# sangminwoo/Temporal-Span-Proposal-Network-VidVRD

Hardware: AMD Instinct MI355X
Metric: tracklet-pairs/sec scored (N=32, T=150, D=2048) (higher is better)
Workload: dtype f32

## Files before the change

### include/tspn_mi355x.h

```cpp
#ifndef TSPN_MI355X_H
#define TSPN_MI355X_H

#include <stddef.h>
#include <stdint.h>

#ifdef __cplusplus
extern "C" {
#endif

#define TSPN_ABI_VERSION 7

enum {
  TSPN_OK = 0,
  TSPN_EINVAL = -1,
  TSPN_EUNSUPPORTED = -2,
  TSPN_EWORKSPACE = -3,
  TSPN_ELAUNCH = -4,
  TSPN_EDEVICE = -5
};

#define TSPN_STATUS_WORDS 16
enum {
  TSPN_STATUS_FAULT = 0,
  TSPN_STATUS_FAULT_INFO = 1,
// ... 62 lines not shown
int tspn_traj_iou_tail_f64(const double* a, const int32_t* len_a, const double* b, int64_t U, int64_t N,
                           int64_t L, float* out, void* stream);

int tspn_pair_index_i64(int64_t N, int64_t base, int64_t* pairs, void* stream);

int tspn_pair_gather_f32(const float* feats, const float* boxes, int64_t NT, int64_t T,
                         int64_t D, const int64_t* pairs, int64_t P,
                         float* out_feat, float* out_geom, void* stream);

int tspn_pack_conv3_f32(const float* W, int64_t M, int64_t Cin, int64_t split,
                        float* packed, void* stream);

int tspn_conv3_f32(const float* x, int64_t B, int64_t Cin, int64_t T,
                   const float* packed, int64_t M, const float* bias, int relu,
                   float* y, void* stream);

int tspn_conv3_tc_f32(const float* x, int64_t B, int64_t T, int64_t Cin,
                      const float* packed, int64_t M, const float* bias, int relu,
                      float* y, void* stream);

int tspn_pack_conv3_wino63_frag_f32(const float* W, int64_t M, int64_t Cin, int64_t split, float* frag,
                                    void* stream);
size_t tspn_conv3_tc_wino63_workspace_bytes(int64_t B, int64_t T, int64_t Cin);
int tspn_conv3_tc_wino63_f32(const float* x, int64_t B, int64_t T, int64_t Cin, const float* frag,
                             int64_t M, const float* bias, int relu, float* y,
                             void* workspace, size_t workspace_bytes, void* stream);
int tspn_conv3_tc_wino63_set_piece_form(int form);

size_t tspn_pack_conv3_wino63_f16x3_elements(int64_t M, int64_t Cin, int64_t split);
int tspn_pack_conv3_wino63_f16x3(const float* W, int64_t M, int64_t Cin, int64_t split, int16_t* packed, void* stream);
size_t tspn_conv3_tc_wino63_f16x3_workspace_bytes(int64_t B, int64_t T, int64_t Cin, int64_t M);
int tspn_conv3_tc_wino63_f16x3(const float* x, int64_t B, int64_t T, int64_t Cin, const int16_t* packed,
                               int64_t M, const float* bias, int relu, float* y,
                               void* workspace, size_t workspace_bytes, void* stream);
int tspn_conv3_tc_wino63_f16x3_set_tail_split(int on);
int tspn_conv3_tc_wino63_f16x3_input_form(int64_t NT, int64_t T, int64_t Cin, int cus);
int tspn_conv3_tc_wino63_f16x3_set_input_form(int form);
int tspn_conv3_tc_wino63_f16x3_input(const float* x, int64_t B, int64_t T, int64_t Cin, int64_t M, void* split_input,
                                     size_t split_input_bytes, float* fbar, uint64_t* hot_slots, void* stream);


int tspn_heads_f32(int mode, const float* a, const float* b, int64_t lda,
                   const int64_t* ia, const int64_t* ib, int64_t idx_stride, const float* bias,
                   const float* Wh, const float* bh, int64_t H,
                   int64_t P, int64_t C, int64_t T, float* out, void* stream);

int tspn_heads_pairgrid_f32(const float* y, int64_t B, int64_t N, int64_t C, int64_t T,
                            const float* Wh, const float* bh, int64_t H, float* out,
                            void* stream);

size_t tspn_heads_pairgrid_f16x3_split_bytes(int64_t C, int64_t H);
int tspn_heads_pairgrid_f16x3_set_force_exact(int on);
int tspn_heads_pair_f16x3_set_diag_skip(int on);
int tspn_heads_pairgrid_f16x3(const float* y, int64_t ldt, int64_t B, int64_t N, int64_t C, int64_t T,
                              const float* Wh, const float* bh, int64_t H, void* split_buf, size_t split_bytes,
                              float* out, void* stream);

int tspn_temporal_mean_f32(const float* x, int64_t R, int64_t T, int64_t Cdim,
                           int layout_tc, float* out, void* stream);
int tspn_temporal_sum_f32(const float* x, int64_t R, int64_t T, int64_t Cdim, float* out, void* stream);

int tspn_pair_rows_f32(const float* src, int64_t NT, int64_t D, const int64_t* pairs,
                       int64_t P, float* out, void* stream);

int tspn_transpose_td_f32(const float* x, int64_t R, int64_t T, int64_t D, float* out,
                          void* stream);

size_t tspn_decode_topk_workspace_bytes(int64_t S, int64_t P, int64_t topk_pair);
int tspn_decode_topk_f32(const float* rel_logit, const int64_t* pairs,
                         const float* cls_sub, const float* cls_obj, int64_t ld,
                         int64_t seg_rows, int64_t row_mul, int64_t S, int64_t P, int64_t K,
                         int64_t NO, int64_t topk_pair, int64_t topk_seg,
                         float* out_score, int64_t* out_triplet, int64_t* out_pair_tid,
                         void* workspace, size_t workspace_bytes, void* stream);

int tspn_decode_spans_f32(const float* heads, int64_t P, int64_t A, int64_t T,
                          const float* sizes_host, int64_t top_k, double nms_threshold,
                          int64_t pre_nms, int64_t* out_anchor, int64_t* out_span,
                          float* out_span_f, float* out_score, int64_t* out_count, void* stream);

typedef struct tspn_fused_desc {
  int64_t B, N, T, D;
  int64_t A, K;
  const float* feats;
  const int64_t* pairs;
  int64_t P;
  int64_t canonical_pairs;
  const float* conv_packed;
  int64_t conv_algo;
  const float* conv_bias;
  const float* head_w;
  const float* head_b;
  const float* cls_w;
  const float* cls_b;
  float* out_heads;
  float* out_logits;
  void* workspace;
  size_t workspace_bytes;
  void* ev_conv_begin;
  void* ev_conv_end;
  void* ev_logits_ready;
  const float* conv_weight;
  int64_t conv_check;
} tspn_fused_desc;

size_t tspn_forward_fused_workspace_bytes(const tspn_fused_desc* d);
// ... 210 lines not shown
```

### temporal-span-proposal-network-vidvrd_amd/_abi.py

```python
import ctypes
import os
import re
import threading

HERE = os.path.dirname(os.path.abspath(__file__))
ROOT = os.path.dirname(HERE)
LIB_PATH = os.environ.get("TSPN_LIB_PATH") or os.path.join(HERE, "libtspn_mi355x.so")
HEADER_PATH = os.path.join(ROOT, "include", "tspn_mi355x.h")

ABI_VERSION = 7
TSPN_OK = 0
TSPN_EINVAL = -1
TSPN_EUNSUPPORTED = -2
TSPN_EWORKSPACE = -3
TSPN_ELAUNCH = -4
TSPN_EDEVICE = -5
STATUS_WORDS = 16
STATUS_FAULT, STATUS_FAULT_INFO, STATUS_CONV_ERR, STATUS_CONV_CHECKS = 0, 1, 2, 3
FAULT_HANDOVER = 1
CONV_CHECK_HOT_OFFSET, CONV_CHECK_SCRATCH_BYTES = 256, 256 + 256 * 64
GEOM_CHANNELS = 8
CONV_DIRECT, CONV_WINOGRAD63, CONV_WINOGRAD63_F16X3 = 0, 1, 2

_c_f32p = ctypes.c_void_p
# ... 18 lines not shown
        ("conv_weight", _vp), ("conv_check", _i64),
    ]


class FusedBf16Desc(ctypes.Structure):
    _fields_ = [
        ("B", _i64), ("N", _i64), ("T", _i64), ("D", _i64),
        ("A", _i64), ("K", _i64),
        ("feats", _vp), ("pairs", _vp), ("P", _i64),
        ("conv_packed", _vp), ("conv_bias", _vp),
        ("head_packed", _vp), ("head_b", _vp),
        ("cls_w", _vp), ("cls_b", _vp),
        ("out_heads", _vp), ("out_logits", _vp),
        ("workspace", _vp), ("workspace_bytes", _sz),
        ("ev_conv_begin", _vp), ("ev_conv_end", _vp), ("ev_logits_ready", _vp),
    ]


PROTOTYPES = {
    "tspn_version": (_int, []),
    "tspn_fused_desc_size": (_sz, []),
    "tspn_fused_bf16_desc_size": (_sz, []),
    "tspn_last_error": (ctypes.c_char_p, []),
    "tspn_error_string": (ctypes.c_char_p, [_int]),
    "tspn_status_attach": (_int, [_vp]),
    "tspn_status_fault": (_int, []),
    "tspn_status_clear": (_int, []),
    "tspn_status_selftest": (_int, [_vp, _vp]),
    "tspn_conv3_spot_check_f32": (_int, [_vp, _i64, _i64, _i64, _vp, _i64, _i64, _i64, _vp, _int, _vp, _i64, _vp, _i64, _vp]),
    "tspn_predicate_head_workspace_bytes": (_sz, [_i64, _i64, _i64]),
    "tspn_predicate_head_f32": (_int, [_vp, _i64, _i64, _i64, _vp, _vp, _i64, _vp, _int, _vp, _sz, _vp]),
    "tspn_predicate_head_norm_workspace_bytes": (_sz, [_i64, _i64, _i64, _i64, _i64, _i64]),
    "tspn_predicate_head_norm_f32": (_int, [_vp, _i64, _i64, _i64, _vp, _vp, _i64, _i64, _i64, _i64, _vp, _int,
                                            _vp, _sz, _vp]),
    "tspn_feature_preprocess_f32": (_int, [_vp, _i64, _i64, _i64, _i64, _i64, _i64, _vp]),
    "tspn_proposal_pair_filter_i64": (_int, [_vp, _vp, _vp, _vp, _i64, _vp, _vp, _vp, _vp]),
    "tspn_gather_rows_f32": (_int, [_vp, _i64, _i64, _vp, _i64, _i64, _vp, _vp]),
    "tspn_ppn_pair_matrix_topk_f32": (_int, [_vp, _i64, _i64, _i64, _i64, _i64,
                                             _vp, _vp, _vp, _vp, _vp, _vp, _vp, _vp,
                                             _i64, _vp, _vp, _vp]),
    "tspn_traj_iou_f32": (_int, [_vp, _i64, _vp, _i64, _i64, _i64, _vp, _vp]),
    "tspn_traj_iou_tail_f64": (_int, [_vp, _vp, _vp, _i64, _i64, _i64, _vp, _vp]),
    "tspn_pair_index_i64": (_int, [_i64, _i64, _vp, _vp]),
    "tspn_pair_gather_f32": (_int, [_vp, _vp, _i64, _i64, _i64, _vp, _i64, _vp, _vp, _vp]),
    "tspn_pack_conv3_f32": (_int, [_vp, _i64, _i64, _i64, _vp, _vp]),
    "tspn_conv3_f32": (_int, [_vp, _i64, _i64, _i64, _vp, _i64, _vp, _int, _vp, _vp]),
    "tspn_conv3_tc_f32": (_int, [_vp, _i64, _i64, _i64, _vp, _i64, _vp, _int, _vp, _vp]),
    "tspn_heads_f32": (_int, [_int, _vp, _vp, _i64, _vp, _vp, _i64, _vp, _vp, _vp, _i64, _i64, _i64,
                              _i64, _vp, _vp]),
    "tspn_heads_pairgrid_f32": (_int, [_vp, _i64, _i64, _i64, _i64, _vp, _vp, _i64, _vp, _vp]),
    "tspn_heads_pairgrid_f16x3_split_bytes": (_sz, [_i64, _i64]),
    "tspn_heads_pairgrid_f16x3_set_force_exact": (_int, [_int]),
    "tspn_heads_pair_f16x3_set_diag_skip": (_int, [_int]),
    "tspn_heads_pairgrid_f16x3": (_int, [_vp, _i64, _i64, _i64, _i64, _i64, _vp, _vp, _i64, _vp, _sz, _vp, _vp]),
    "tspn_temporal_mean_f32": (_int, [_vp, _i64, _i64, _i64, _int, _vp, _vp]),
    "tspn_temporal_sum_f32": (_int, [_vp, _i64, _i64, _i64, _vp, _vp]),
    "tspn_pair_rows_f32": (_int, [_vp, _i64, _i64, _vp, _i64, _vp, _vp]),
    "tspn_transpose_td_f32": (_int, [_vp, _i64, _i64, _i64, _vp, _vp]),
    "tspn_decode_topk_workspace_bytes": (_sz, [_i64, _i64, _i64]),
    "tspn_decode_topk_f32": (_int, [_vp, _vp, _vp, _vp, _i64, _i64, _i64, _i64, _i64, _i64, _i64, _i64, _i64,
                                    _vp, _vp, _vp, _vp, _sz, _vp]),
    "tspn_decode_spans_f32": (_int, [_vp, _i64, _i64, _i64, ctypes.POINTER(ctypes.c_float), _i64,
                                     ctypes.c_double, _i64, _vp, _vp, _vp, _vp, _vp, _vp]),
    "tspn_forward_fused_workspace_bytes": (_sz, [ctypes.POINTER(FusedDesc)]),
    "tspn_forward_fused_f32": (_int, [ctypes.POINTER(FusedDesc), _vp]),
    "tspn_temporal_encoder_heads_f32": (_int, [_vp, _i64, _i64, _i64, _vp, _vp, _vp, _vp, _i64,
                                               _vp, _vp, _vp]),
    "tspn_pack_conv2d_f32": (_int, [_vp, _i64, _i64, _i64, _i64, _vp, _vp]),
    "tspn_conv2d_nhwc_f32": (_int, [_vp, _i64, _i64, _i64, _i64, _vp, _i64, _i64, _i64, _i64, _i64, _vp, _vp,
                                    _int, _vp, _vp]),
    "tspn_pack_conv2d_frag_f32": (_int, [_vp, _i64, _i64, _i64, _i64, _vp, _vp]),
    "tspn_conv2d_nhwc_frag_f32": (_int, [_vp, _i64, _i64, _i64, _i64, _vp, _i64, _i64, _i64, _i64, _i64, _vp, _vp,
                                         _int, _vp, _vp]),
    "tspn_pack_conv2d_frag_bf16": (_int, [_vp, _i64, _i64, _i64, _i64, _vp, _vp]),
    "tspn_conv2d_nhwc_bf16": (_int, [_vp, _i64, _i64, _i64, _i64, _vp, _i64, _i64, _i64, _i64, _i64, _vp, _vp,
                                     _int, _vp, _vp]),
    "tspn_roi_align_nhwc_f32": (_int, [_vp, _i64, _i64, _i64, _i64, _vp, _i64, _i64, ctypes.c_float, _int, _int,
                                       _int, _vp, _vp]),
    "tspn_pack_conv2d_frag_cin4_f32": (_int, [_vp, _i64, _i64, _i64, _i64, _vp, _vp]),
    "tspn_conv2d_nhwc_cin4_f32": (_int, [_vp, _i64, _i64, _i64, _vp, _i64, _i64, _i64, _i64, _i64, _vp, _int, _vp, _vp]),
    "tspn_max_pool_nhwc_f32": (_int, [_vp, _i64, _i64, _i64, _i64, _i64, _i64, _i64, _vp, _int, _vp]),
    "tspn_bottleneck_tail_bf16": (_int, [_vp, _i64, _i64, _i64, _i64, _vp, _vp, _vp, _vp, _vp, _vp, _vp]),
    "tspn_bottleneck_block_bf16": (_int, [_vp, _i64, _i64, _i64, _i64, _vp, _vp, _vp, _vp, _vp, _vp, _vp, _vp]),
    "tspn_bottleneck_block_proj_bf16": (_int, [_vp, _i64, _i64, _i64, _i64, _i64, _i64, _vp, _vp, _vp, _vp, _vp, _vp, _vp, _vp,
                                               _vp, _vp]),
    "tspn_bottleneck_block_res_bf16": (_int, [_vp, _i64, _i64, _i64, _i64, _i64, _i64, _vp, _vp, _vp, _vp, _vp, _vp, _vp, _vp, _vp]),
    "tspn_bottleneck_tail_io_bf16": (_int, [_vp, _i64, _i64, _i64, _i64, _vp, _vp, _vp, _vp, _vp, _vp, _vp]),
    "tspn_bottleneck_tail_pipe_bf16": (_int, [_vp, _i64, _i64, _i64, _i64, _vp, _vp, _vp, _vp, _vp, _vp, _i64, _vp]),
    "tspn_bottleneck_tail_next_bf16": (_int, [_vp, _i64, _i64, _i64, _i64, _vp, _vp, _vp, _vp, _vp, _vp, _vp, _vp, _vp, _vp]),
    "tspn_stem_bf16_workspace_bytes": (_sz, [_i64, _i64, _i64]),
    "tspn_pack_stem_bf16": (_int, [_vp, _i64, _vp, _vp]),
    "tspn_stem_conv_bf16": (_int, [_vp, _i64, _i64, _i64, _vp, _i64, _vp, _vp, _sz, _vp, _vp]),
    "tspn_max_pool_nhwc_bf16": (_int, [_vp, _i64, _i64, _i64, _i64, _i64, _i64, _i64, _vp, _vp]),
    "tspn_stem_pool_bf16": (_int, [_vp, _i64, _i64, _i64, _vp, _i64, _vp, _vp, _sz, _vp, _vp]),
    "tspn_roi_align_nhwc_bf16": (_int, [_vp, _i64, _i64, _i64, _i64, _vp, _i64, _i64, ctypes.c_float, _int, _int,
                                        _int, _vp, _vp]),
    "tspn_roi_align_nhwc_f32_bf16out": (_int, [_vp, _i64, _i64, _i64, _i64, _vp, _i64, _i64, ctypes.c_float, _int, _int,
                                               _int, _vp, _vp]),
    "tspn_pack_conv3_wino63_frag_f32": (_int, [_vp, _i64, _i64, _i64, _vp, _vp]),
    "tspn_conv3_tc_wino63_workspace_bytes": (_sz, [_i64, _i64, _i64]),
    "tspn_conv3_tc_wino63_f32": (_int, [_vp, _i64, _i64, _i64, _vp, _i64, _vp, _int, _vp, _vp, _sz, _vp]),
    "tspn_conv3_tc_wino63_set_piece_form": (_int, [_int]),
    "tspn_pack_conv3_wino63_f16x3_elements": (_sz, [_i64, _i64, _i64]),
    "tspn_pack_conv3_wino63_f16x3": (_int, [_vp, _i64, _i64, _i64, _vp, _vp]),
    "tspn_conv3_tc_wino63_f16x3_workspace_bytes": (_sz, [_i64, _i64, _i64, _i64]),
    "tspn_conv3_tc_wino63_f16x3": (_int, [_vp, _i64, _i64, _i64, _vp, _i64, _vp, _int, _vp, _vp, _sz, _vp]),
# ... 103 lines not shown
```

### temporal-span-proposal-network-vidvrd_amd/csrc/pairf16/tspn_heads_pair_f16x3.hip

```cpp
#include "tspn_common.h"
#include "tspn_device.h"

#include <type_traits>

namespace {
using namespace tspn_dev;

constexpr int PF_S = 8, PF_O = 8, PF_T = 32, PF_CK = 32;
constexpr int PF_ROWS = PF_S + PF_O;
constexpr int PF_STAGE = PF_ROWS * PF_CK * PF_T;
constexpr int PF_THREADS = 64 * PF_S;
constexpr size_t PF_SMEM = sizeof(float) * 2 * PF_STAGE;
constexpr int PF_HDR_BYTES = 256;
constexpr int PF_KSTEP_BYTES = 2 * 64 * 16;
constexpr float PF_LO = 2048.f, PF_LO_INV = 1.f / 2048.f;
constexpr float PF_RANGE = 16384.f;

typedef _Float16 f16x2 __attribute__((ext_vector_type(2)));

std::atomic<int> g_force_exact{0};
std::atomic<int> g_diag_skip{1};

__device__ __forceinline__ unsigned split_lo(unsigned h2, float as0, float as1) {
  unsigned d;
  const float neg = -PF_LO;
  asm("v_fma_mixlo_f16 %0, %1, %2, %3 op_sel_hi:[1,0,0]" : "=v"(d) : "v"(h2), "s"(neg), "v"(as0));
  asm("v_fma_mixhi_f16 %0, %1, %2, %3 op_sel:[1,0,0] op_sel_hi:[1,0,0]" : "+v"(d) : "v"(h2), "s"(neg), "v"(as1));
  return d;
}

__global__ __launch_bounds__(1024) void pairf16_scale_kernel(const float* __restrict__ Wh, int C, int H,
                                                            unsigned* __restrict__ hdr) {
  __shared__ unsigned bad_s[16];
  const int lane = threadIdx.x & 63, h = threadIdx.x >> 6;
  float mx = 0.f;
  bool finite = true;
  auto take = [&](float w, float& m) {
    const float a = fabsf(w);
    finite = finite && (a < __builtin_inff());
    m = fmaxf(m, a);
  };
  if (h < H && (reinterpret_cast<uintptr_t>(Wh) & 15) == 0) {
    const float4* row = reinterpret_cast<const float4*>(Wh + (int64_t)h * C);
    const int n4 = C >> 2;
    float m[4] = {0.f, 0.f, 0.f, 0.f};
    int c = lane;
    for (; c + 192 < n4; c += 256) {
      float4 v[4];
#pragma unroll
      for (int u = 0; u < 4; ++u) v[u] = row[c + 64 * u];
#pragma unroll
      for (int u = 0; u < 4; ++u) { take(v[u].x, m[u]); take(v[u].y, m[u]); take(v[u].z, m[u]); take(v[u].w, m[u]); }
    }
    for (; c < n4; c += 64) {
      const float4 v = row[c];
      take(v.x, m[0]); take(v.y, m[0]); take(v.z, m[0]); take(v.w, m[0]);
    }
    mx = fmaxf(fmaxf(m[0], m[1]), fmaxf(m[2], m[3]));
  } else if (h < H) {
    for (int c = lane; c < C; c += 64) take(Wh[(int64_t)h * C + c], mx);
  }
#pragma unroll
  for (int o = 32; o > 0; o >>= 1) mx = fmaxf(mx, __shfl_xor(mx, o, 64));
  const bool all_finite = __all(finite);
  int e = 0;
  (void)frexpf(mx, &e);
  const bool bad = h < H && (!all_finite || !(mx >= 0x1p-100f) || e > 100);
  if (lane == 0) {
    bad_s[h] = bad ? 1u : 0u;
    hdr[1 + h] = __float_as_uint((h < H && !bad) ? ldexpf(1.f, e) : 1.f);
  }
  __syncthreads();
  if (threadIdx.x == 0) {
    unsigned f = 0;
    for (int i = 0; i < 16; ++i) f |= bad_s[i];
    hdr[0] = f;
  }
  if (threadIdx.x >= 17 && threadIdx.x < PF_HDR_BYTES / 4) hdr[threadIdx.x] = 0;
}

__global__ __launch_bounds__(64) void pairf16_pack_kernel(const float* __restrict__ Wh, int C, int H,
                                                         const unsigned* __restrict__ hdr, u32x4* __restrict__ frag) {
  const int lane = threadIdx.x, h = lane & 15, kg = lane >> 4;
  const float scale = 1.f / __uint_as_float(hdr[1 + h]);
  unsigned hi[4], lo[4];
#pragma unroll
  for (int ip = 0; ip < 4; ++ip) {
    f16x2 wh, wl;
#pragma unroll
    for (int e = 0; e < 2; ++e) {
      const int c = blockIdx.x * PF_CK + kg + 4 * (2 * ip + e);
      const float w = (h < H) ? Wh[(int64_t)h * C + c] * scale : 0.f;
      const _Float16 a = (_Float16)w;
      wh[e] = a;
      wl[e] = (_Float16)((w - (float)a) * PF_LO);
    }
    hi[ip] = __builtin_bit_cast(unsigned, wh);
    lo[ip] = __builtin_bit_cast(unsigned, wl);
  }
  frag[(int64_t)blockIdx.x * 128 + lane] = u32x4{hi[0], hi[1], hi[2], hi[3]};
  frag[(int64_t)blockIdx.x * 128 + 64 + lane] = u32x4{lo[0], lo[1], lo[2], lo[3]};
}

__device__ __noinline__ void exact_tile(const float* __restrict__ y, int64_t ldt, int C, int T, int N, int H,
                                        const float* __restrict__ Wh, const float* __restrict__ bh,
                                        float* __restrict__ out, int64_t b, int sb, int ob, int t0) {
  const int t = t0 + (threadIdx.x & 31);
  if (t >= T) return;
  for (int idx = threadIdx.x >> 5; idx < PF_S * PF_O * H; idx += PF_THREADS / 32) {
    const int pair = idx / H, h = idx - pair * H;
    const int s = sb * PF_S + (pair >> 3), o = ob * PF_O + (pair & 7);
    if (s >= N || o >= N || s == o) continue;
    const float* up = y + ((b * N + s) * 2 * (int64_t)C) * ldt + t;
    const float* vp = y + ((b * N + o) * 2 * (int64_t)C + C) * ldt + t;
    const float* w = Wh + (int64_t)h * C;
    float sum = 0.f;
    for (int c = 0; c < C; ++c) sum = __builtin_fmaf(w[c], tspn::relu_f32(up[c * ldt] + vp[c * ldt]), sum);
    const int64_t p = b * N * (int64_t)(N - 1) + (int64_t)s * (N - 1) + o - (o > s ? 1 : 0);
    out[(p * H + h) * (int64_t)T + t] = sum + (bh ? bh[h] : 0.f);
  }
}

__global__ __launch_bounds__(PF_THREADS, 1) void heads_pair_f16x3_kernel(
    const float* __restrict__ y, int64_t ldt, int C, int T, int N, int H, const float* __restrict__ Wh,
    const float* __restrict__ bh, const unsigned* __restrict__ hdr, const u32x4* __restrict__ frag,
    float* __restrict__ out, int ntb, int nob, int nsb, int64_t ngroups, int force_exact, int diag_skip) {
  extern __shared__ __attribute__((aligned(16))) char smem_raw[];
  float* S = reinterpret_cast<float*>(smem_raw);

  const int tid = threadIdx.x;
  const int lane = tid & 63;
  const int wave = __builtin_amdgcn_readfirstlane(tid >> 6);
  const int j = lane & 15, kg = lane >> 4;
  int sb, ob;
  const int64_t G = pair_stage_group(blockIdx.x, nsb, nob, sb, ob);
  if (G >= ngroups) return;
  const int64_t b = G / ntb;
  const int t0 = (int)(G - b * ntb) * PF_T;
  const int64_t rowlen = 2 * (int64_t)C * ldt;

  if (force_exact | (int)hdr[0]) {
    exact_tile(y, ldt, C, T, N, H, Wh, bh, out, b, sb, ob, t0);
    return;
  }

  const __amdgpu_buffer_rsrc_t rsrc_y = buffer_rsrc(y + b * N * rowlen, (int)(unsigned)((int64_t)N * rowlen * 4));
  unsigned voff[2];
  const unsigned loff = (unsigned)((lane >> 3) * ldt + min((int64_t)t0 + (lane & 7) * 4, ldt - 4));
#pragma unroll
  for (int r = 0; r < 2; ++r) {
    const int row = 2 * wave + r;
    const int local = row < PF_S ? sb * PF_S + row : ob * PF_O + (row - PF_S);
    const int64_t trk = min(local, N - 1);
    voff[r] = (unsigned)((trk * rowlen + (row < PF_S ? 0 : (int64_t)C * ldt) + loff) * 4);
  }
  const int piece_bytes = (int)(8 * ldt * 4);
  int y_soff = 0;
  auto stage = [&](int buf) {
#pragma unroll
    for (int r = 0; r < 2; ++r) {
#pragma unroll
      for (int q = 0; q < 4; ++q)
        bglds16(rsrc_y, voff[r], y_soff + q * piece_bytes, S + buf * PF_STAGE + ((2 * wave + r) * PF_CK + 8 * q) * PF_T);
    }
    y_soff += 4 * piece_bytes;
  };

  f32x4 acc_hi[PF_O][2], acc_lo[PF_O][2];
#pragma unroll
  for (int o = 0; o < PF_O; ++o) {
#pragma unroll
    for (int cb = 0; cb < 2; ++cb) acc_hi[o][cb] = acc_lo[o][cb] = f32x4{0.f, 0.f, 0.f, 0.f};
  }

  const int nk = C / PF_CK;
  stage(0);
  u32x4 wh = frag[lane], wl = frag[64 + lane];
  asm volatile("s_waitcnt vmcnt(0)" ::: "memory");
  __syncthreads();
  const float* urow = S + (wave * PF_CK + kg) * PF_T + 2 * j;
  const float* vrow = S + (PF_S * PF_CK + kg) * PF_T + 2 * j;
  const float* trow = vrow + wave * PF_CK * PF_T;
  float mu = 0.f, mv = 0.f;
  const bool diag = diag_skip && sb == ob;
  auto kloop = [&](auto diag_c) {
    constexpr bool DIAG = decltype(diag_c)::value;
    constexpr int NS = DIAG ? PF_O - 1 : PF_O;
    for (int k = 0; k < nk; ++k) {
      const int buf = k & 1;
      u32x4 whn = wh, wln = wl;
      if (k + 1 < nk) {
        stage(buf ^ 1);
        whn = frag[(int64_t)(k + 1) * 128 + lane];
        wln = frag[(int64_t)(k + 1) * 128 + 64 + lane];
      }
// ... 35 lines not shown
#pragma unroll
          for (int cb = 0; cb < 2; ++cb) {
            unsigned ph[4], pl[4];
#pragma unroll
            for (int ip = 0; ip < 4; ++ip) {
              const f16x2 h = __builtin_convertvector(f32x2{a[2 * ip][cb], a[2 * ip + 1][cb]}, f16x2);
              ph[ip] = __builtin_bit_cast(unsigned, h);
              pl[ip] = split_lo(ph[ip], as[2 * ip][cb], as[2 * ip + 1][cb]);
            }
            gh[cb] = u32x4{ph[0], ph[1], ph[2], ph[3]};
            gl[cb] = u32x4{pl[0], pl[1], pl[2], pl[3]};
          }
        }
        if (o > 0) {
          const f16x8 h0 = __builtin_bit_cast(f16x8, fh[0]), h1 = __builtin_bit_cast(f16x8, fh[1]);
          const f16x8 l0 = __builtin_bit_cast(f16x8, fl[0]), l1 = __builtin_bit_cast(f16x8, fl[1]);
          acc_hi[o - 1][0] = __builtin_amdgcn_mfma_f32_16x16x32_f16(a_hi, h0, acc_hi[o - 1][0], 0, 0, 0);
          acc_lo[o - 1][0] = __builtin_amdgcn_mfma_f32_16x16x32_f16(a_hi, l0, acc_lo[o - 1][0], 0, 0, 0);
          acc_hi[o - 1][1] = __builtin_amdgcn_mfma_f32_16x16x32_f16(a_hi, h1, acc_hi[o - 1][1], 0, 0, 0);
          acc_lo[o - 1][1] = __builtin_amdgcn_mfma_f32_16x16x32_f16(a_hi, l1, acc_lo[o - 1][1], 0, 0, 0);
          acc_lo[o - 1][0] = __builtin_amdgcn_mfma_f32_16x16x32_f16(a_lo, h0, acc_lo[o - 1][0], 0, 0, 0);
          acc_lo[o - 1][1] = __builtin_amdgcn_mfma_f32_16x16x32_f16(a_lo, h1, acc_lo[o - 1][1], 0, 0, 0);
        }
        if (o > 0 && o < NS) {
#define TSPN_G                                         \
  __builtin_amdgcn_sched_group_barrier(0x008, 1, 0);   \
  __builtin_amdgcn_sched_group_barrier(0x100, 2, 0);   \
  __builtin_amdgcn_sched_group_barrier(0x002, 10, 0);
          TSPN_G TSPN_G TSPN_G TSPN_G TSPN_G TSPN_G
#undef TSPN_G
        }
        __builtin_amdgcn_sched_barrier(0);
#pragma unroll
        for (int cb = 0; cb < 2; ++cb) {
          fh[cb] = gh[cb];
          fl[cb] = gl[cb];
        }
#pragma unroll
        for (int i = 0; i < 8; ++i) v[i] = vn[i];
      }
      wh = whn;
      wl = wln;
      asm volatile("s_waitcnt vmcnt(0)" ::: "memory");
      __syncthreads();
    }
  };
  if (diag) kloop(std::true_type{});
  else kloop(std::false_type{});

  const int tA = t0 + 2 * j;
  const int s = sb * PF_S + wave;
  const bool bad = tA < T && ((s < N && !(mu <= PF_RANGE)) || (ob * PF_O + wave < N && !(mv <= PF_RANGE)));
  if (__syncthreads_or(bad)) {
    exact_tile(y, ldt, C, T, N, H, Wh, bh, out, b, sb, ob, t0);
    return;
  }

  if (tA >= T || s >= N) return;
  float inv[4], bias[4];
#pragma unroll
  for (int r = 0; r < 4; ++r) {
    const int h = 4 * kg + r;
    inv[r] = __uint_as_float(hdr[1 + h]);
    bias[r] = (h < H && bh) ? bh[h] : 0.f;
  }
#pragma unroll
  for (int o = 0; o < PF_O; ++o) {
    if (diag && o == PF_O - 1) continue;
    const int ot = ob * PF_O + (diag ? (wave + 1 + o) & 7 : o);
    if (ot >= N || ot == s) continue;
    const int64_t p = b * N * (int64_t)(N - 1) + (int64_t)s * (N - 1) + ot - (ot > s ? 1 : 0);
#pragma unroll
    for (int r = 0; r < 4; ++r) {
      const int h = 4 * kg + r;
      if (h >= H) continue;
      const float v0 = __builtin_fmaf(acc_lo[o][0][r], PF_LO_INV, acc_hi[o][0][r]) * inv[r] + bias[r];
      const float v1 = __builtin_fmaf(acc_lo[o][1][r], PF_LO_INV, acc_hi[o][1][r]) * inv[r] + bias[r];
      *reinterpret_cast<float2*>(out + (p * H + h) * (int64_t)T + tA) = make_float2(v0, v1);
    }
  }
}

}

size_t tspn::heads_pair_f16x3_split_bytes(int64_t C, int64_t H) {
  if (C <= 0 || C % PF_CK != 0 || C >= (1 << 24) || H <= 0 || H > 16) return 0;
  return (size_t)PF_HDR_BYTES + (size_t)(C / PF_CK) * PF_KSTEP_BYTES;
}

bool tspn::heads_pair_f16x3_supported(const float* y, int64_t ldt, int64_t N, int64_t C, int64_t T, int64_t H,
                                      const float* out) {
  return H > 0 && H <= 16 && C > 0 && C % PF_CK == 0 && C < (1 << 24) && T > 0 && T % 2 == 0 && ldt >= T && ldt % 4 == 0 &&
         ldt < (1 << 24) && N < (1 << 15) && N * 2 * C * ldt * 4 < (1LL << 31) && tspn::aligned16(y) &&
         (reinterpret_cast<uintptr_t>(out) & 7) == 0;
}

int tspn::heads_pair_f16x3(const float* y, int64_t ldt, int64_t B, int64_t N, int64_t C, int64_t T, const float* Wh,
                           const float* bh, int64_t H, void* split_buf, size_t split_bytes, float* out, void* stream) {
  const char* what = "tspn_heads_pairgrid_f16x3";
  TSPN_REQUIRE(B >= 0 && N >= 0 && C > 0 && T > 0 && ldt >= T, TSPN_EINVAL,
               "%s: bad sizes B=%lld N=%lld C=%lld T=%lld ldt=%lld", what, (long long)B, (long long)N, (long long)C,
               (long long)T, (long long)ldt);
  TSPN_REQUIRE(H > 0 && H <= 16, TSPN_EUNSUPPORTED, "%s: H=%lld not in [1,16]", what, (long long)H);
  if (B == 0 || N < 2) return TSPN_OK;
  TSPN_REQUIRE(y && Wh && out && split_buf, TSPN_EINVAL, "%s: null pointer", what);
  TSPN_REQUIRE(tspn::heads_pair_f16x3_supported(y, ldt, N, C, T, H, out), TSPN_EUNSUPPORTED,
               "%s: needs C %% 32 == 0, even T, ldt %% 4 == 0, a video's projections below 2 GB, y 16-byte and out 8-byte "
               "aligned", what);
  const size_t need = tspn::heads_pair_f16x3_split_bytes(C, H);
  TSPN_REQUIRE(split_bytes >= need, TSPN_EWORKSPACE, "%s: split buffer %zu < %zu bytes", what, split_bytes, need);
  TSPN_REQUIRE(tspn::aligned16(split_buf), TSPN_EINVAL, "%s: split buffer must be 16-byte aligned", what);
  const int ntb = (int)tspn::ceil_div(T, PF_T);
  const int nsb = (int)tspn::ceil_div(N, PF_S), nob = (int)tspn::ceil_div(N, PF_O);
  const int64_t ngroups = B * ntb;
  const int64_t nwg = tspn::ceil_div(ngroups, 8) * 8 * nsb * nob;
  TSPN_REQUIRE(nwg < (1LL << 31), TSPN_EUNSUPPORTED, "%s: grid too large", what);
  hipStream_t s = TSPN_STREAM(stream);
  unsigned* hdr = static_cast<unsigned*>(split_buf);
  u32x4* frag = reinterpret_cast<u32x4*>(static_cast<char*>(split_buf) + PF_HDR_BYTES);
  hipLaunchKernelGGL(pairf16_scale_kernel, dim3(1), dim3(1024), 0, s, Wh, (int)C, (int)H, hdr);
  hipLaunchKernelGGL(pairf16_pack_kernel, dim3((unsigned)(C / PF_CK)), dim3(64), 0, s, Wh, (int)C, (int)H, hdr, frag);
  static tspn::LdsLimit lds;
  if (int rc = lds.ensure(reinterpret_cast<const void*>(heads_pair_f16x3_kernel), PF_SMEM, what)) return rc;
  hipLaunchKernelGGL(heads_pair_f16x3_kernel, dim3((unsigned)nwg), dim3(PF_THREADS), PF_SMEM, s, y, ldt, (int)C, (int)T,
                     (int)N, (int)H, Wh, bh, hdr, frag, out, ntb, nob, nsb, ngroups,
                     g_force_exact.load(std::memory_order_relaxed), g_diag_skip.load(std::memory_order_relaxed));
  return tspn::check_launch(what);
}

extern "C" size_t tspn_heads_pairgrid_f16x3_split_bytes(int64_t C, int64_t H) {
  return tspn::heads_pair_f16x3_split_bytes(C, H);
}

extern "C" int tspn_heads_pairgrid_f16x3_set_force_exact(int on) {
  TSPN_REQUIRE(on == 0 || on == 1, TSPN_EINVAL, "tspn_heads_pairgrid_f16x3_set_force_exact: on must be 0 or 1");
  return g_force_exact.exchange(on, std::memory_order_relaxed);
}

extern "C" int tspn_heads_pair_f16x3_set_diag_skip(int on) {
  TSPN_REQUIRE(on == 0 || on == 1, TSPN_EINVAL, "tspn_heads_pair_f16x3_set_diag_skip: on must be 0 or 1");
  return g_diag_skip.exchange(on, std::memory_order_relaxed);
}

extern "C" int tspn_heads_pairgrid_f16x3(const float* y, int64_t ldt, int64_t B, int64_t N, int64_t C, int64_t T,
                                         const float* Wh, const float* bh, int64_t H, void* split_buf, size_t split_bytes,
                                         float* out, void* stream) {
  return tspn::heads_pair_f16x3(y, ldt, B, N, C, T, Wh, bh, H, split_buf, split_bytes, out, stream);
}
```

### temporal-span-proposal-network-vidvrd_amd/ops.py

```python
import ctypes
import threading

import torch

from . import _abi

__all__ = [
    "predicate_head", "feature_preprocess_", "ppn_pair_matrix_topk", "traj_iou", "traj_iou_tail", "pair_index",
    "pair_gather", "pack_conv3", "conv3", "conv3_tc", "pack_conv3_wino63", "conv3_tc_wino63", "pack_conv3_wino63_f16x3", "conv3_tc_wino63_f16x3", "heads", "heads_pairgrid", "heads_pairgrid_f16x3", "heads_pairgrid_f16x3_split_bytes",
    "heads_pairgrid_f16x3_set_force_exact", "heads_pair_f16x3_set_diag_skip","temporal_mean", "temporal_sum", "pair_rows", "transpose_td",
    "forward_fused", "temporal_encoder_heads", "fused_workspace_bytes", "fused_bf16_workspace_bytes", "decode_topk", "decode_spans", "decode_span_relations",
    "span_anchor_labels", "span_loss", "span_anchor_sample", "pair_labels", "span_match",
    "cast_bf16", "pack_conv3_bf16", "pack_heads_bf16", "conv3_tc_bf16", "heads_pairgrid_bf16",
    "pair_plan", "heads_pairlist_bf16",
    "transpose_cast_bf16", "temporal_encoder_heads_bf16",
    "temporal_mean_bf16", "forward_fused_bf16", "span_predicate",
    "pack_span_cls_bf16", "span_predicate_bf16", "decode_span_relations_bf16", "bottleneck_block_bf16", "bottleneck_block_proj_bf16", "bottleneck_block_res_bf16",
    "proposal_pair_filter", "gather_rows", "wino63_set_piece_form", "wino63_f16x3_set_tail_split", "conv3_spot_check",
    "wino63_f16x3_set_input_form", "wino63_f16x3_input_form", "wino63_f16x3_input",
    "pack_conv2d", "pack_conv2d_frag", "conv2d_nhwc", "roi_align_nhwc", "pack_conv2d_frag_bf16", "conv2d_nhwc_bf16", "max_pool_nhwc", "pack_conv2d_frag_cin4", "conv2d_nhwc_cin4", "max_pool_nhwc_bf16", "pack_stem_bf16", "stem_conv_bf16", "stem_pool_bf16", "bottleneck_tail_bf16",
    "eval_traj_volume", "eval_viou", "eval_greedy_match", "evalobj_tiou", "evalobj_claim",
    "status_words", "status_fault", "status_clear", "status_selftest",
]


_status_blocks = {}
_status_lock = threading.Lock()


def _status_block(index=None):
    idx = torch.cuda.current_device() if index is None else int(index)
    blk = _status_blocks.get(idx)
    if blk is not None:
        return blk
    with _status_lock:
        blk = _status_blocks.get(idx)
        if blk is None:
            raw = torch.zeros(_abi.STATUS_WORDS + 16, dtype=torch.int32).pin_memory()
            off = (-(raw.data_ptr() // 4)) % 16
            blk = raw[off:off + _abi.STATUS_WORDS]
            with torch.cuda.device(idx):
                _abi.check(_abi.lib().tspn_status_attach(ctypes.c_void_p(blk.data_ptr())))
            blk = _status_blocks[idx] = blk.numpy()
    return blk


def _stream():
    blk = _status_block()
    fault = int(blk[_abi.STATUS_FAULT])
    if fault:
        raise _abi.TspnError(_abi.TSPN_EDEVICE,
                             f"device {torch.cuda.current_device()} reported fault 0x{fault:x}"
                             + (" (an LDS hand-over between waves timed out)" if fault & _abi.FAULT_HANDOVER else "")
                             + f", info 0x{int(blk[_abi.STATUS_FAULT_INFO]) & 0xffffffff:x}, in an earlier launch of this library: "
                             "results produced since are not to be trusted; ops.status_clear() re-arms")
    return ctypes.c_void_p(torch.cuda.current_stream().cuda_stream)


def status_words(device=None):
    return _status_block(None if device is None else torch.device(device).index)


def status_fault(device=None):
# ... 427 lines not shown
    nsp2 = -(-(B * (-(-T // 6))) // 256) * 256
    vbytes = 8 * 2 * Cin * nsp2 * 2
    v = workspace[:vbytes].view(torch.int16).view(8, 2, Cin // 8, nsp2, 8)
    eoff = -(-vbytes // 256) * 256
    e = workspace[eoff:eoff + 8 * nsp2 * 4].view(torch.int32).view(8, nsp2)
    return v, e, fbar, (slots[:, 0].max() if hot else None)


def heads(a, head_w, head_b, b=None, ia=None, ib=None, bias=None, channels=None, num_pairs=None):
    _dev(a, "a"); _dev(head_w, "head_w")
    mode = 0 if b is None else 1
    lda, T = a.shape[1], a.shape[2]
    C = channels if channels is not None else lda
    H = head_w.shape[0]
    if head_w.shape[1] != C:
        raise ValueError("heads: head_w / channel mismatch")
    for nm, t in (("ia", ia), ("ib", ib)):
        if t is not None:
            _dev(t, nm, torch.int64)
    if b is not None:
        _dev(b, "b")
        if b.shape[1:] != a.shape[1:]:
            raise ValueError("heads: a / b shape mismatch")
    if num_pairs is None:
        num_pairs = ia.shape[0] if ia is not None else a.shape[0]
    out = torch.empty((num_pairs, H, T), dtype=torch.float32, device=a.device)
    _abi.check(_abi.lib().tspn_heads_f32(mode, _p(a), _p(b), lda, _p(ia), _p(ib), 1, _p(bias),
                                         _p(head_w), _p(head_b), H, num_pairs, C, T, _p(out), _stream()))
    return out


def heads_pairgrid(y, B, N, head_w, head_b):
    _dev(y, "y"); _dev(head_w, "head_w")
    NT, C2, T = y.shape
    C, H = C2 // 2, head_w.shape[0]
    if NT != B * N or head_w.shape[1] != C:
        raise ValueError("heads_pairgrid: shape mismatch")
    out = torch.empty((B * N * max(N - 1, 0), H, T), dtype=torch.float32, device=y.device)
    _abi.check(_abi.lib().tspn_heads_pairgrid_f32(_p(y), B, N, C, T, _p(head_w), _p(head_b), H, _p(out),
                                                  _stream()))
    return out


def heads_pairgrid_f16x3_split_bytes(C, H):
    return int(_abi.lib().tspn_heads_pairgrid_f16x3_split_bytes(int(C), int(H)))


def heads_pairgrid_f16x3_set_force_exact(on):
    return _toggle("tspn_heads_pairgrid_f16x3_set_force_exact", on)


def heads_pair_f16x3_set_diag_skip(on):
    return _toggle("tspn_heads_pair_f16x3_set_diag_skip", on)


def heads_pairgrid_f16x3(y, B, N, head_w, head_b, T=None, split_buf=None, out=None):
    _dev(y, "y"); _dev(head_w, "head_w")
    NT, C2, ldt = y.shape
    T = ldt if T is None else int(T)
    C, H = C2 // 2, head_w.shape[0]
    if NT != B * N or head_w.shape[1] != C:
        raise ValueError("heads_pairgrid_f16x3: shape mismatch")
    if split_buf is None:
        split_buf = _ws(heads_pairgrid_f16x3_split_bytes(C, H), y.device)
    if out is None:
        out = torch.empty((B * N * max(N - 1, 0), H, T), dtype=torch.float32, device=y.device)
    _abi.check(_abi.lib().tspn_heads_pairgrid_f16x3(_p(y), ldt, B, N, C, T, _p(head_w), _p(head_b), H, _p(split_buf),
                                                    split_buf.numel(), _p(out), _stream()))
    return out


def temporal_mean(x, layout_tc):
    _dev(x, "x")
    if layout_tc:
        R, T, Cd = x.shape
    else:
        R, Cd, T = x.shape
    out = torch.empty((R, Cd), dtype=torch.float32, device=x.device)
    _abi.check(_abi.lib().tspn_temporal_mean_f32(_p(x), R, T, Cd, 1 if layout_tc else 0, _p(out), _stream()))
    return out


def temporal_sum(x):
    _dev(x, "x")
    R, T, Cd = x.shape
    out = torch.empty((R, Cd), dtype=torch.float32, device=x.device)
    _abi.check(_abi.lib().tspn_temporal_sum_f32(_p(x), R, T, Cd, _p(out), _stream()))
    return out


def pair_rows(src, pairs):
    _dev(src, "src"); _dev(pairs, "pairs", torch.int64)
    NT, D = src.shape
    P = pairs.shape[0]
    out = torch.empty((P, 2 * D), dtype=torch.float32, device=src.device)
    _abi.check(_abi.lib().tspn_pair_rows_f32(_p(src), NT, D, _p(pairs), P, _p(out), _stream()))
    return out


def transpose_td(x):
    _dev(x, "x")
    R, T, D = x.shape
    out = torch.empty((R, D, T), dtype=torch.float32, device=x.device)
    _abi.check(_abi.lib().tspn_transpose_td_f32(_p(x), R, T, D, _p(out), _stream()))
    return out

# ... 1111 lines not shown
```

Measured before the change: 1.252 million.

## Add 16-wave pair-head kernel form splitting object tiles across two half-blocks

Adds a second kernel form that launches 1024 threads per workgroup instead of 512, with the object tile split between two halves of waves (each handling 4 of the 8 object tracklets), sharing the staged subject/object rows in LDS. A heuristic picks this form when C>=1024 and the tile count is moderate, which aims to increase per-CU wave parallelism and cut per-wave MFMA chains when there are few tiles. It also switches the lo-split scaling to a packed f32 multiply and adds a vote-based exact fallback. Costs are extra LDS for a vote word, more waves contending for LDS bandwidth, and added code complexity.

```diff
diff --git a/include/tspn_mi355x.h b/include/tspn_mi355x.h
--- a/include/tspn_mi355x.h
+++ b/include/tspn_mi355x.h
@@ -138,6 +138,8 @@
 size_t tspn_heads_pairgrid_f16x3_split_bytes(int64_t C, int64_t H);
 int tspn_heads_pairgrid_f16x3_set_force_exact(int on);
 int tspn_heads_pair_f16x3_set_diag_skip(int on);
+int tspn_heads_pair_f16x3_form(int64_t B, int64_t N, int64_t C, int64_t T);
+int tspn_heads_pair_f16x3_set_form(int form);
 int tspn_heads_pairgrid_f16x3(const float* y, int64_t ldt, int64_t B, int64_t N, int64_t C, int64_t T,
                               const float* Wh, const float* bh, int64_t H, void* split_buf, size_t split_bytes,
                               float* out, void* stream);
diff --git a/temporal-span-proposal-network-vidvrd_amd/_abi.py b/temporal-span-proposal-network-vidvrd_amd/_abi.py
--- a/temporal-span-proposal-network-vidvrd_amd/_abi.py
+++ b/temporal-span-proposal-network-vidvrd_amd/_abi.py
@@ -94,6 +94,8 @@
     "tspn_heads_pairgrid_f16x3_split_bytes": (_sz, [_i64, _i64]),
     "tspn_heads_pairgrid_f16x3_set_force_exact": (_int, [_int]),
     "tspn_heads_pair_f16x3_set_diag_skip": (_int, [_int]),
+    "tspn_heads_pair_f16x3_form": (_int, [_i64, _i64, _i64, _i64]),
+    "tspn_heads_pair_f16x3_set_form": (_int, [_int]),
     "tspn_heads_pairgrid_f16x3": (_int, [_vp, _i64, _i64, _i64, _i64, _i64, _vp, _vp, _i64, _vp, _sz, _vp, _vp]),
     "tspn_temporal_mean_f32": (_int, [_vp, _i64, _i64, _i64, _int, _vp, _vp]),
     "tspn_temporal_sum_f32": (_int, [_vp, _i64, _i64, _i64, _vp, _vp]),
diff --git a/temporal-span-proposal-network-vidvrd_amd/csrc/pairf16/tspn_heads_pair_f16x3.hip b/temporal-span-proposal-network-vidvrd_amd/csrc/pairf16/tspn_heads_pair_f16x3.hip
--- a/temporal-span-proposal-network-vidvrd_amd/csrc/pairf16/tspn_heads_pair_f16x3.hip
+++ b/temporal-span-proposal-network-vidvrd_amd/csrc/pairf16/tspn_heads_pair_f16x3.hip
@@ -13,6 +13,7 @@
 constexpr size_t PF_SMEM = sizeof(float) * 2 * PF_STAGE;
 constexpr int PF_HDR_BYTES = 256;
 constexpr int PF_KSTEP_BYTES = 2 * 64 * 16;
+constexpr size_t PF_SMEM16 = PF_SMEM + 2 * PF_KSTEP_BYTES + 16;
 constexpr float PF_LO = 2048.f, PF_LO_INV = 1.f / 2048.f;
 constexpr float PF_RANGE = 16384.f;
 
@@ -20,6 +21,7 @@
 
 std::atomic<int> g_force_exact{0};
 std::atomic<int> g_diag_skip{1};
+std::atomic<int> g_form{0};
 
 __device__ __forceinline__ unsigned split_lo(unsigned h2, float as0, float as1) {
   unsigned d;
@@ -27,6 +29,12 @@
   asm("v_fma_mixlo_f16 %0, %1, %2, %3 op_sel_hi:[1,0,0]" : "=v"(d) : "v"(h2), "s"(neg), "v"(as0));
   asm("v_fma_mixhi_f16 %0, %1, %2, %3 op_sel:[1,0,0] op_sel_hi:[1,0,0]" : "+v"(d) : "v"(h2), "s"(neg), "v"(as1));
   return d;
+}
+
+__device__ __forceinline__ f32x2 pk_scale_lo(f32x2 a) {
+  const f32x2 c = f32x2{PF_LO, PF_LO};
+  asm("v_pk_mul_f32 %0, %0, %1" : "+v"(a) : "s"(c));
+  return a;
 }
 
 __global__ __launch_bounds__(1024) void pairf16_scale_kernel(const float* __restrict__ Wh, int C, int H,
@@ -104,10 +112,11 @@
 
 __device__ __noinline__ void exact_tile(const float* __restrict__ y, int64_t ldt, int C, int T, int N, int H,
                                         const float* __restrict__ Wh, const float* __restrict__ bh,
-                                        float* __restrict__ out, int64_t b, int sb, int ob, int t0) {
-  const int t = t0 + (threadIdx.x & 31);
+                                        float* __restrict__ out, int64_t b, int sb, int ob, int t0, int tid,
+                                        int nthreads) {
+  const int t = t0 + (tid & 31);
   if (t >= T) return;
-  for (int idx = threadIdx.x >> 5; idx < PF_S * PF_O * H; idx += PF_THREADS / 32) {
+  for (int idx = tid >> 5; idx < PF_S * PF_O * H; idx += nthreads >> 5) {
     const int pair = idx / H, h = idx - pair * H;
     const int s = sb * PF_S + (pair >> 3), o = ob * PF_O + (pair & 7);
     if (s >= N || o >= N || s == o) continue;
@@ -121,10 +130,181 @@
   }
 }
 
-__global__ __launch_bounds__(PF_THREADS, 1) void heads_pair_f16x3_kernel(
+__device__ __forceinline__ void pair_tile_w16(const float* __restrict__ y, int64_t ldt, int C, int T, int N, int H,
+                                              const float* __restrict__ Wh, const float* __restrict__ bh,
+                                              const unsigned* __restrict__ hdr, const u32x4* __restrict__ frag,
+                                              float* __restrict__ out, int ntb, int nob, int nsb, int64_t ngroups,
+                                              int force_exact, int diag_skip) {
+  extern __shared__ __attribute__((aligned(16))) char smem_raw[];
+  float* S = reinterpret_cast<float*>(smem_raw);
+  constexpr int OW = PF_O / 2;
+
+  const int tid = threadIdx.x;
+  const int lane = tid & 63;
+  const int wave = __builtin_amdgcn_readfirstlane(tid >> 6);
+  const int sw = wave & 7, hf = wave >> 3;
+  const int j = lane & 15, kg = lane >> 4;
+  int sb, ob;
+  const int64_t G = pair_stage_group(blockIdx.x, nsb, nob, sb, ob);
+  if (G >= ngroups) return;
+  const int64_t b = G / ntb;
+  const int t0 = (int)(G - b * ntb) * PF_T;
+  const int64_t rowlen = 2 * (int64_t)C * ldt;
+
+  if (force_exact | (int)hdr[0]) {
+    exact_tile(y, ldt, C, T, N, H, Wh, bh, out, b, sb, ob, t0, tid, 2 * PF_THREADS);
+    return;
+  }
+
+  const __amdgpu_buffer_rsrc_t rsrc_y = buffer_rsrc(y + b * N * rowlen, (int)(unsigned)((int64_t)N * rowlen * 4));
+  const unsigned loff = (unsigned)((lane >> 3) * ldt + min((int64_t)t0 + (lane & 7) * 4, ldt - 4));
+  const int local = wave < PF_S ? sb * PF_S + wave : ob * PF_O + (wave - PF_S);
+  const int64_t trk = min(local, N - 1);
+  const unsigned voff = (unsigned)((trk * rowlen + (wave < PF_S ? 0 : (int64_t)C * ldt) + loff) * 4);
+  const int piece_bytes = (int)(8 * ldt * 4);
+  const int nk = C / PF_CK;
+  const __amdgpu_buffer_rsrc_t rsrc_w = buffer_rsrc(frag, nk * PF_KSTEP_BYTES);
+  char* Wf = smem_raw + PF_SMEM;
+  int y_soff = 0, w_soff = 0;
+  auto stage = [&](int buf) {
+#pragma unroll
+    for (int q = 0; q < 4; ++q)
+      bglds16(rsrc_y, voff, y_soff + q * piece_bytes, S + buf * PF_STAGE + (wave * PF_CK + 8 * q) * PF_T);
+    y_soff += 4 * piece_bytes;
+    if (sw == 0) {
+      const unsigned l16 = 16u * __builtin_amdgcn_mbcnt_hi(~0u, __builtin_amdgcn_mbcnt_lo(~0u, 0u));
+      bglds16(rsrc_w, l16, w_soff + hf * 1024, Wf + buf * PF_KSTEP_BYTES + hf * 1024);
+    }
+    w_soff += PF_KSTEP_BYTES;
+  };
+
+  f32x4 acc_hi[OW][2], acc_lo[OW][2];
+#pragma unroll
+  for (int o = 0; o < OW; ++o) {
+#pragma unroll
+    for (int cb = 0; cb < 2; ++cb) acc_hi[o][cb] = acc_lo[o][cb] = f32x4{0.f, 0.f, 0.f, 0.f};
+  }
+
+  unsigned* vote = reinterpret_cast<unsigned*>(Wf + 2 * PF_KSTEP_BYTES);
+  if (tid == 0) *vote = 0;
+  stage(0);
+  asm volatile("s_waitcnt vmcnt(0)" ::: "memory");
+  __syncthreads();
+  const float* urow = S + (sw * PF_CK + kg) * PF_T + 2 * j;
+  const float* vrow = S + ((PF_S + OW * hf) * PF_CK + kg) * PF_T + 2 * j;
+  float m = 0.f;
+  const bool diag = diag_skip && sb == ob;
+  const bool own = diag && (sw >> 2) == hf;
+  const int ns = own ? OW - 1 : OW;
+  const int rot = own ? (sw & 3) + 1 : 0;
+  auto kloop = [&](auto diag_c) {
+    constexpr bool DIAG = decltype(diag_c)::value;
+    for (int k = 0; k < nk; ++k) {
+      const int buf = k & 1;
+      if (k + 1 < nk) stage(buf ^ 1);
+      const float* ub = urow + buf * PF_STAGE;
+      const float* vb = vrow + buf * PF_STAGE;
+      const float* tb = ub + PF_S * PF_CK * PF_T;
+      f32x2 u[8];
+#pragma unroll
+      for (int i = 0; i < 8; ++i) u[i] = *reinterpret_cast<const f32x2*>(ub + 4 * i * PF_T);
+      if (hf == 0) {
+#pragma unroll
+        for (int i = 0; i < 8; ++i)
+          m = __builtin_elementwise_maximum(__builtin_elementwise_maximum(m, __builtin_fabsf(u[i][0])), __builtin_fabsf(u[i][1]));
+      } else {
+#pragma unroll
+        for (int i = 0; i < 8; ++i) {
+          const f32x2 vt = *reinterpret_cast<const f32x2*>(tb + 4 * i * PF_T);
+          m = __builtin_elementwise_maximum(__builtin_elementwise_maximum(m, __builtin_fabsf(vt[0])), __builtin_fabsf(vt[1]));
+        }
+      }
+      const u32x4* wf = reinterpret_cast<const u32x4*>(Wf + buf * PF_KSTEP_BYTES) + lane;
+#pragma unroll
+      for (int o = 0; o < OW; ++o) {
+        if (DIAG && o == OW - 1 && ns < OW) continue;
+        const float* vp = vb + (DIAG ? ((rot + o) & 3) : o) * (PF_CK * PF_T);
+        unsigned ph[2][4], pl[2][4];
+#pragma unroll
+        for (int ip = 0; ip < 4; ++ip) {
+          const f32x2 x0 = u[2 * ip] + *reinterpret_cast<const f32x2*>(vp + 4 * (2 * ip) * PF_T);
+          const f32x2 x1 = u[2 * ip + 1] + *reinterpret_cast<const f32x2*>(vp + 4 * (2 * ip + 1) * PF_T);
+          const f32x2 a0 = f32x2{tspn::relu_f32(x0[0]), tspn::relu_f32(x0[1])};
+          const f32x2 a1 = f32x2{tspn::relu_f32(x1[0]), tspn::relu_f32(x1[1])};
+#pragma unroll
+          for (int cb = 0; cb < 2; ++cb)
+            ph[cb][ip] = __builtin_bit_cast(unsigned, __builtin_convertvector(f32x2{a0[cb], a1[cb]}, f16x2));
+          const f32x2 as0 = pk_scale_lo(a0), as1 = pk_scale_lo(a1);
+#pragma unroll
+          for (int cb = 0; cb < 2; ++cb) pl[cb][ip] = split_lo(ph[cb][ip], as0[cb], as1[cb]);
+          if (ip == 1) __builtin_amdgcn_sched_barrier(0);
+        }
+        const f16x8 h0 = __builtin_bit_cast(f16x8, u32x4{ph[0][0], ph[0][1], ph[0][2], ph[0][3]});
+        const f16x8 h1 = __builtin_bit_cast(f16x8, u32x4{ph[1][0], ph[1][1], ph[1][2], ph[1][3]});
+        const f16x8 l0 = __builtin_bit_cast(f16x8, u32x4{pl[0][0], pl[0][1], pl[0][2], pl[0][3]});
+        const f16x8 l1 = __builtin_bit_cast(f16x8, u32x4{pl[1][0], pl[1][1], pl[1][2], pl[1][3]});
+        const f16x8 a_hi = __builtin_bit_cast(f16x8, wf[0]);
+        acc_hi[o][0] = __builtin_amdgcn_mfma_f32_16x16x32_f16(a_hi, h0, acc_hi[o][0], 0, 0, 0);
+        acc_lo[o][0] = __builtin_amdgcn_mfma_f32_16x16x32_f16(a_hi, l0, acc_lo[o][0], 0, 0, 0);
+        acc_hi[o][1] = __builtin_amdgcn_mfma_f32_16x16x32_f16(a_hi, h1, acc_hi[o][1], 0, 0, 0);
+        acc_lo[o][1] = __builtin_amdgcn_mfma_f32_16x16x32_f16(a_hi, l1, acc_lo[o][1], 0, 0, 0);
+        const f16x8 a_lo = __builtin_bit_cast(f16x8, wf[64]);
+        acc_lo[o][0] = __builtin_amdgcn_mfma_f32_16x16x32_f16(a_lo, h0, acc_lo[o][0], 0, 0, 0);
+        acc_lo[o][1] = __builtin_amdgcn_mfma_f32_16x16x32_f16(a_lo, h1, acc_lo[o][1], 0, 0, 0);
+        __builtin_amdgcn_sched_barrier(0);
+      }
+      asm volatile("s_waitcnt vmcnt(0)" ::: "memory");
+      __syncthreads();
+    }
+  };
+  if (diag) kloop(std::true_type{});
+  else kloop(std::false_type{});
+
+  const int lane_e = __builtin_amdgcn_mbcnt_hi(~0u, __builtin_amdgcn_mbcnt_lo(~0u, 0u));
+  const int tA = t0 + 2 * (lane_e & 15);
+  const int kg_e = lane_e >> 4;
+  const int s = sb * PF_S + sw;
+  if (tA < T && local < N && !(m <= PF_RANGE)) *vote = 1;
+  __syncthreads();
+  if (*vote) {
+    exact_tile(y, ldt, C, T, N, H, Wh, bh, out, b, sb, ob, t0, wave * 64 + lane_e, 2 * PF_THREADS);
+    return;
+  }
+
+  if (tA >= T || s >= N) return;
+  float inv[4], bias[4];
+#pragma unroll
+  for (int r = 0; r < 4; ++r) {
+    const int h = 4 * kg_e + r;
+    inv[r] = __uint_as_float(hdr[1 + h]);
+    bias[r] = (h < H && bh) ? bh[h] : 0.f;
+  }
+#pragma unroll
+  for (int o = 0; o < OW; ++o) {
+    if (o >= ns) continue;
+    const int ot = ob * PF_O + OW * hf + ((rot + o) & 3);
+    if (ot >= N || ot == s) continue;
+    const int64_t p = b * N * (int64_t)(N - 1) + (int64_t)s * (N - 1) + ot - (ot > s ? 1 : 0);
+#pragma unroll
+    for (int r = 0; r < 4; ++r) {
+      const int h = 4 * kg_e + r;
+      if (h >= H) continue;
+      const float v0 = __builtin_fmaf(acc_lo[o][0][r], PF_LO_INV, acc_hi[o][0][r]) * inv[r] + bias[r];
+      const float v1 = __builtin_fmaf(acc_lo[o][1][r], PF_LO_INV, acc_hi[o][1][r]) * inv[r] + bias[r];
+      *reinterpret_cast<float2*>(out + (p * H + h) * (int64_t)T + tA) = make_float2(v0, v1);
+    }
+  }
+}
+
+template <int FORM>
+__global__ __launch_bounds__(FORM == 2 ? 2 * PF_THREADS : PF_THREADS, 1) void heads_pair_f16x3_kernel(
     const float* __restrict__ y, int64_t ldt, int C, int T, int N, int H, const float* __restrict__ Wh,
     const float* __restrict__ bh, const unsigned* __restrict__ hdr, const u32x4* __restrict__ frag,
     float* __restrict__ out, int ntb, int nob, int nsb, int64_t ngroups, int force_exact, int diag_skip) {
+  if constexpr (FORM == 2) {
+    pair_tile_w16(y, ldt, C, T, N, H, Wh, bh, hdr, frag, out, ntb, nob, nsb, ngroups, force_exact, diag_skip);
+    return;
+  }
   extern __shared__ __attribute__((aligned(16))) char smem_raw[];
   float* S = reinterpret_cast<float*>(smem_raw);
 
@@ -140,7 +320,7 @@
   const int64_t rowlen = 2 * (int64_t)C * ldt;
 
   if (force_exact | (int)hdr[0]) {
-    exact_tile(y, ldt, C, T, N, H, Wh, bh, out, b, sb, ob, t0);
+    exact_tile(y, ldt, C, T, N, H, Wh, bh, out, b, sb, ob, t0, tid, PF_THREADS);
     return;
   }
 
@@ -282,7 +462,7 @@
   const int s = sb * PF_S + wave;
   const bool bad = tA < T && ((s < N && !(mu <= PF_RANGE)) || (ob * PF_O + wave < N && !(mv <= PF_RANGE)));
   if (__syncthreads_or(bad)) {
-    exact_tile(y, ldt, C, T, N, H, Wh, bh, out, b, sb, ob, t0);
+    exact_tile(y, ldt, C, T, N, H, Wh, bh, out, b, sb, ob, t0, tid, PF_THREADS);
     return;
   }
 
@@ -323,6 +503,13 @@
   return H > 0 && H <= 16 && C > 0 && C % PF_CK == 0 && C < (1 << 24) && T > 0 && T % 2 == 0 && ldt >= T && ldt % 4 == 0 &&
          ldt < (1 << 24) && N < (1 << 15) && N * 2 * C * ldt * 4 < (1LL << 31) && tspn::aligned16(y) &&
          (reinterpret_cast<uintptr_t>(out) & 7) == 0;
+}
+
+extern "C" int tspn_heads_pair_f16x3_form(int64_t B, int64_t N, int64_t C, int64_t T) {
+  if (B <= 0 || N < 2 || C <= 0 || T <= 0) return 1;
+  const int64_t nb = tspn::ceil_div(N, PF_S);
+  const int64_t tiles = B * tspn::ceil_div(T, PF_T) * nb * nb;
+  return (C >= 1024 && tiles >= 256 && tiles <= 2560) ? 2 : 1;
 }
 
 int tspn::heads_pair_f16x3(const float* y, int64_t ldt, int64_t B, int64_t N, int64_t C, int64_t T, const float* Wh,
@@ -350,12 +537,25 @@
   u32x4* frag = reinterpret_cast<u32x4*>(static_cast<char*>(split_buf) + PF_HDR_BYTES);
   hipLaunchKernelGGL(pairf16_scale_kernel, dim3(1), dim3(1024), 0, s, Wh, (int)C, (int)H, hdr);
   hipLaunchKernelGGL(pairf16_pack_kernel, dim3((unsigned)(C / PF_CK)), dim3(64), 0, s, Wh, (int)C, (int)H, hdr, frag);
-  static tspn::LdsLimit lds;
-  if (int rc = lds.ensure(reinterpret_cast<const void*>(heads_pair_f16x3_kernel), PF_SMEM, what)) return rc;
-  hipLaunchKernelGGL(heads_pair_f16x3_kernel, dim3((unsigned)nwg), dim3(PF_THREADS), PF_SMEM, s, y, ldt, (int)C, (int)T,
-                     (int)N, (int)H, Wh, bh, hdr, frag, out, ntb, nob, nsb, ngroups,
-                     g_force_exact.load(std::memory_order_relaxed), g_diag_skip.load(std::memory_order_relaxed));
+  int form = g_form.load(std::memory_order_relaxed);
+  if (form == 0) form = tspn_heads_pair_f16x3_form(B, N, C, T);
+  const int fe = g_force_exact.load(std::memory_order_relaxed), ds = g_diag_skip.load(std::memory_order_relaxed);
+  static tspn::LdsLimit lds8, lds16;
+  if (form == 2) {
+    if (int rc = lds16.ensure(reinterpret_cast<const void*>(heads_pair_f16x3_kernel<2>), PF_SMEM16, what)) return rc;
+    hipLaunchKernelGGL(heads_pair_f16x3_kernel<2>, dim3((unsigned)nwg), dim3(2 * PF_THREADS), PF_SMEM16, s, y, ldt, (int)C,
+                       (int)T, (int)N, (int)H, Wh, bh, hdr, frag, out, ntb, nob, nsb, ngroups, fe, ds);
+  } else {
+    if (int rc = lds8.ensure(reinterpret_cast<const void*>(heads_pair_f16x3_kernel<1>), PF_SMEM, what)) return rc;
+    hipLaunchKernelGGL(heads_pair_f16x3_kernel<1>, dim3((unsigned)nwg), dim3(PF_THREADS), PF_SMEM, s, y, ldt, (int)C,
+                       (int)T, (int)N, (int)H, Wh, bh, hdr, frag, out, ntb, nob, nsb, ngroups, fe, ds);
+  }
   return tspn::check_launch(what);
+}
+
+extern "C" int tspn_heads_pair_f16x3_set_form(int form) {
+  TSPN_REQUIRE(form >= 0 && form <= 2, TSPN_EINVAL, "tspn_heads_pair_f16x3_set_form: form must be 0, 1 or 2");
+  return g_form.exchange(form, std::memory_order_relaxed);
 }
 
 extern "C" size_t tspn_heads_pairgrid_f16x3_split_bytes(int64_t C, int64_t H) {
diff --git a/temporal-span-proposal-network-vidvrd_amd/ops.py b/temporal-span-proposal-network-vidvrd_amd/ops.py
--- a/temporal-span-proposal-network-vidvrd_amd/ops.py
+++ b/temporal-span-proposal-network-vidvrd_amd/ops.py
@@ -8,7 +8,7 @@
 __all__ = [
     "predicate_head", "feature_preprocess_", "ppn_pair_matrix_topk", "traj_iou", "traj_iou_tail", "pair_index",
     "pair_gather", "pack_conv3", "conv3", "conv3_tc", "pack_conv3_wino63", "conv3_tc_wino63", "pack_conv3_wino63_f16x3", "conv3_tc_wino63_f16x3", "heads", "heads_pairgrid", "heads_pairgrid_f16x3", "heads_pairgrid_f16x3_split_bytes",
-    "heads_pairgrid_f16x3_set_force_exact", "heads_pair_f16x3_set_diag_skip","temporal_mean", "temporal_sum", "pair_rows", "transpose_td",
+    "heads_pairgrid_f16x3_set_force_exact", "heads_pair_f16x3_set_diag_skip", "heads_pair_f16x3_set_form", "heads_pair_f16x3_form", "temporal_mean", "temporal_sum", "pair_rows", "transpose_td",
     "forward_fused", "temporal_encoder_heads", "fused_workspace_bytes", "fused_bf16_workspace_bytes", "decode_topk", "decode_spans", "decode_span_relations",
     "span_anchor_labels", "span_loss", "span_anchor_sample", "pair_labels", "span_match",
     "cast_bf16", "pack_conv3_bf16", "pack_heads_bf16", "conv3_tc_bf16", "heads_pairgrid_bf16",
@@ -542,6 +542,14 @@
 
 def heads_pair_f16x3_set_diag_skip(on):
     return _toggle("tspn_heads_pair_f16x3_set_diag_skip", on)
+
+
+def heads_pair_f16x3_set_form(form):
+    return _toggle("tspn_heads_pair_f16x3_set_form", form)
+
+
+def heads_pair_f16x3_form(B, N, C, T):
+    return int(_abi.lib().tspn_heads_pair_f16x3_form(int(B), int(N), int(C), int(T)))
 
 
 def heads_pairgrid_f16x3(y, B, N, head_w, head_b, T=None, split_buf=None, out=None):
```

Result: no change. 1.264 million, median of 6 (+1.0%).
